# limix/CellRegMap

Hardware: AMD Instinct MI355X
Metric: variant-tests/sec (interaction test) (higher is better)
Workload: dtype f64

## Files before the change

cellregmap_amd/csrc/api_core.hip:

```cpp
#include <dlfcn.h>

#include <algorithm>
#include <atomic>
#include <cstdarg>
#include <mutex>

#include <map>

#include "crm_internal.h"
#include "eigh.h"

namespace crm {

static thread_local std::string g_error;

void set_error(const char* fmt, ...) {
    char buf[1024];
    va_list ap;
    va_start(ap, fmt);
    vsnprintf(buf, sizeof buf, fmt, ap);
    va_end(ap);
    g_error = buf;
}

// ... 220 lines not shown
}

int crm_ctx_synchronize(crm_ctx* c) {
    return crm::guarded_on("crm_ctx_synchronize", c, [&]() -> int {
    if (!c) return CRM_ERR_ARG;
    CRM_HIP(hipSetDevice(c->device));
    CRM_HIP(hipStreamSynchronize(c->stream));
    return CRM_OK;
    });
}

int crm_set_block_variants(crm_ctx* c, int variants) {
    return crm::guarded_on("crm_set_block_variants", c, [&]() -> int {
    if (!c || variants < 0) return CRM_ERR_ARG;
    c->block_variants = variants == 0 ? 0 : (int)round_up(variants, 128);
    return CRM_OK;
    });
}

int crm_set_null_fit_polish(crm_ctx* c, int on) {
    return crm::guarded_on("crm_set_null_fit_polish", c, [&]() -> int {
    if (!c) return CRM_ERR_ARG;
    c->polish = on != 0;
    return CRM_OK;
    });
}

int crm_set_progress_callback(crm_ctx* c, void (*callback)(long, long, void*), void* user) {
    return crm::guarded_on("crm_set_progress_callback", c, [&]() -> int {
    if (!c) return CRM_ERR_ARG;
    if (callback) c->progress[std::this_thread::get_id()] = crm_ctx::Progress{callback, user};
    else c->progress.erase(std::this_thread::get_id());
    return CRM_OK;
    });
}

int crm_set_fast_rotation(crm_ctx* c, int on) {
    return crm::guarded_on("crm_set_fast_rotation", c, [&]() -> int {
    if (!c) return CRM_ERR_ARG;
    c->fast_T = on != 0;
    return CRM_OK;
    });
}

extern "C++" {
namespace crm {
namespace {
struct FormSlot { const char* name; int value; bool set; };
FormSlot g_forms[] = {{"gram_staged", 0, false}, {"kr_no_tail", 0, false}, {"nullfit_per_wave", 0, false}, {"kin_fold", 0, false},
                      {"eigh_one_stage", 0, false}, {"nullfit_exact", 0, false}, {"donor_pairs", 0, false},
                      {"pairs_without_kinship_term", 0, false}, {"flat_kappa_milli", 0, false}, {"chase_abort", 0, false}, {"nullfit_one_per_wave", 0, false},
                      {"kin_diag", 0, false}, {"donor_pairs_rotate", 0, false}, {"rho0_positions", 0, false},
                      {"rotation_tails", 0, false}, {"woodbury_ytY", 0, false},
                      {"wb_block_order", 0, false}, {"block_fused", 0, false}, {"wb_gram_fused", 0, false}};
std::mutex g_forms_mu;
}
int form(const char* name, int otherwise) {
    std::lock_guard<std::mutex> lock(g_forms_mu);
    for (const FormSlot& f : g_forms)
        if (strcmp(f.name, name) == 0) return f.set ? f.value : otherwise;
    return otherwise;
}
}
}

int crm_test_set_form(const char* name, int value, int reset) {
    return crm::guarded("crm_test_set_form", [&]() -> int {
    if (!name) return CRM_ERR_ARG;
    std::lock_guard<std::mutex> lock(crm::g_forms_mu);
    for (crm::FormSlot& f : crm::g_forms)
        if (strcmp(f.name, name) == 0) {
            f.value = value;
            f.set = reset == 0;
            return CRM_OK;
        }
    crm::set_error("crm_test_set_form: no kernel form is called '%s'", name);
    return CRM_ERR_ARG;
    });
}

long crm_test_tail_launches(const crm_ctx* ctx) { return ctx ? ctx->tail_launches : -1; }

long crm_test_spectrum_tail_launches(const crm_ctx* ctx) { return ctx ? ctx->spectrum_tail_launches : -1; }

long crm_test_dense_repeats(const crm_ctx* ctx) { return ctx ? ctx->dense_repeats : -1; }

long crm_test_donor_pair_blocks(const crm_ctx* ctx) { return ctx ? ctx->donor_pair_blocks : -1; }

int crm_test_gram_dma_launches(const crm_ctx* ctx, long* launches) {
    return crm::guarded("crm_test_gram_dma_launches", [&]() -> int {
    if (!ctx || !launches) return CRM_ERR_ARG;
    *launches = ctx->gram_dma_launches;
    return CRM_OK;
    });
}
int crm_test_unrelated_donor_blocks(const crm_ctx* ctx, long* blocks) {
    return crm::guarded("crm_test_unrelated_donor_blocks", [&]() -> int {
    if (!ctx || !blocks) return CRM_ERR_ARG;
    *blocks = ctx->unrelated_donor_blocks;
    return CRM_OK;
    });
}

int crm_test_fused_blocks(const crm_ctx* ctx, long* blocks) {
    return crm::guarded("crm_test_fused_blocks", [&]() -> int {
    if (!ctx || !blocks) return CRM_ERR_ARG;
    *blocks = ctx->fused_blocks;
// ... 346 lines not shown
```

cellregmap_amd/csrc/assemble.hip:

```cpp
#include <type_traits>

#include "nullfit.h"

namespace crm {

namespace {

constexpr int CH = 64;
constexpr int SLD = 66;

typedef double v4d __attribute__((ext_vector_type(4)));

template <int NTL, int NG = 1>
__global__ __launch_bounds__(256) void gram_ext_kernel(AssembleArgs a, double* __restrict__ Gext, int KT) {
    constexpr int ROWS = 16 * NTL, NTILES = NTL * (NTL + 1) / 2, NLOC = (NTILES + NG - 1) / NG, MAXT = (NLOC + 3) / 4,
                  RPT = ROWS / 4;
    extern __shared__ double Ss[];
    __shared__ int tile_ij[NTILES];
    __shared__ const double* tail_ptr[ROWS];
    const int b = blockIdx.x;
    const NullFitOut fit = a.fit[b];
    const AssembleRho R = a.rho[fit.rho_index];
    const int r = R.r;
    const double ratio = fit.v0 / fit.v1;
    const long pos = a.sorted_pos[b];
    const double* __restrict__ Arows = pos >= 0 ? a.A + pos * a.k0 * a.ldA : a.A_none;
    const long a_stride = pos >= 0 ? a.ldA : 0;
    const int tid = threadIdx.x;
    const int lane = tid & 63, wave = tid >> 6;
    const int l15 = lane & 15, lq = lane >> 4;
    const int k0 = a.k0, c = a.c;

    for (int e = tid; e < NTILES; e += 256) {
        int ti = 0, rem = e;
        while (rem >= NTL - ti) { rem -= NTL - ti; ti++; }
        tile_ij[e] = ti | ((ti + rem) << 8);
    }
    for (int t = tid; t < KT - k0; t += 256) {
        const double* p;
        if (t < c) p = R.tW + (long)t * R.ldW;
        else if (t == c) p = R.T + (long)b * R.ldT;
        else if (t == c + 1) p = R.ty;
        else p = a.wb_R + (long)(t - c - 2) * a.wb_ldR;
        tail_ptr[t] = p;
    }
    __syncthreads();
    const int grp = NG > 1 ? (int)blockIdx.y : 0;
    const int first = (wave + b) & 3;
    const int nloc = (NTILES - grp + NG - 1) / NG;
    const int ntw = (nloc - first + 3) / 4;
    int t_i[MAXT], t_j[MAXT];
#pragma unroll
    for (int t = 0; t < MAXT; t++) {
        const int idx = grp + NG * (first + 4 * t);
        const int ij = tile_ij[idx < NTILES ? idx : 0];
// ... 231 lines not shown
        const int buf = ch & 1;
        if (ch + 1 < nchunks) {
            issue(ch + 1, buf ^ 1);
            weights(ch + 1, buf ^ 1);
        }
        chunk_mma(buf);
        __syncthreads();
    }
    double* const red = Ss + (wave & 1) * NTILES * 256;
    if (wave >= 2) {
#pragma unroll
        for (int t = 0; t < NTILES; t++)
#pragma unroll
            for (int reg = 0; reg < 4; reg++) red[(t * 4 + reg) * 64 + lane] = acc[t][reg];
    }
    __syncthreads();
    if (wave < 2) {
#pragma unroll
        for (int t = 0; t < NTILES; t++)
#pragma unroll
            for (int reg = 0; reg < 4; reg++) acc[t][reg] += red[(t * 4 + reg) * 64 + lane];
    }
    __syncthreads();
    if (wave == 1) {
#pragma unroll
        for (int t = 0; t < NTILES; t++)
#pragma unroll
            for (int reg = 0; reg < 4; reg++) red[(t * 4 + reg) * 64 + lane] = acc[t][reg];
    }
    __syncthreads();
    if (wave != 0) return;
    double* __restrict__ out = Gext + (long)b * KT * KT;
    int idx = 0;
#pragma unroll
    for (int ti = 0; ti < NTL; ti++) {
#pragma unroll
        for (int tj = ti; tj < NTL; tj++, idx++) {
#pragma unroll
            for (int reg = 0; reg < 4; reg++) {
                const double v = acc[idx][reg] + (Ss + NTILES * 256)[(idx * 4 + reg) * 64 + lane];
                const int row = 16 * ti + lq + 4 * reg, col = 16 * tj + l15;
                if (row < KT && col < KT) {
                    out[(long)row * KT + col] = v;
                    if (ti != tj) out[(long)col * KT + row] = v;
                }
            }
        }
    }
}

constexpr int GRAM_WCH = 32;
constexpr int gram_dma_wide_lds_doubles(int ntl) { return 2 * (16 * ((ntl + 3) / 4)) * GRAM_QLD + 4 * GRAM_WCH; }

template <int NTL>
__global__ __launch_bounds__(256, NTL <= 8 ? 2 : 1) void gram_ext_dma_wide_kernel(AssembleArgs a, double* __restrict__ Gext,
                                                                                  int KT) {
    constexpr int WCH = GRAM_WCH;
    constexpr int SLOTS = 16 * ((NTL + 3) / 4);
    constexpr int NTILES = NTL * (NTL + 1) / 2, MAXT = (NTILES + 3) / 4;
    constexpr int QLD = GRAM_QLD;
    constexpr int BUF = SLOTS * QLD;
    static_assert(gram_dma_wide_lds_doubles(NTL) == 2 * BUF + 4 * WCH, "the launch allocates what the kernel lays out");
    constexpr int IPW = SLOTS / 4;
    extern __shared__ double Ss[];
    double* const dS = Ss + 2 * BUF;
    const int b = blockIdx.x;
    const NullFitOut fit = a.fit[b];
    const AssembleRho R = a.rho[fit.rho_index];
    const int r = R.r;
    const double ratio = fit.v0 / fit.v1;
    const long pos = a.sorted_pos[b];
    const double* __restrict__ Arows = pos >= 0 ? a.A + pos * a.k0 * a.ldA : a.A_none;
    const long a_stride = pos >= 0 ? a.ldA : 0;
    const int tid = threadIdx.x;
    const int lane = tid & 63, wave = __builtin_amdgcn_readfirstlane(tid >> 6);
    const int l15 = lane & 15, lq = lane >> 4;
    const int k0 = a.k0, c = a.c;

    auto row_ptr = [&](int row) -> const double* {
        if (row >= KT) row = 0;
        if (row < k0) return Arows + (long)row * a_stride;
        const int t = row - k0;
        if (t > c + 1) return a.wb_R + (long)(t - c - 2) * a.wb_ldR;
        return t < c ? R.tW + (long)t * R.ldW : (t == c ? R.T + (long)b * R.ldT : R.ty);
    };
    auto row_off = [](int row) { return (16 * (row >> 6) + (row & 15)) * QLD + ((row >> 4) & 3) * WCH; };
    gram_gptr_t src[IPW];
#pragma unroll
    for (int q = 0; q < IPW; q++) {
        const int slot = wave + 4 * q;
        src[q] = (gram_gptr_t)(row_ptr(64 * (slot >> 4) + 16 * lq + (slot & 15)) + 2 * l15);
    }
    const int first = (wave + b) & 3;
    const int ntw = (NTILES - first + 3) / 4;
    int t_i[MAXT], t_j[MAXT], t_ij[MAXT];
#pragma unroll
    for (int t = 0; t < MAXT; t++) {
        int ti = 0, rem = first + 4 * t < NTILES ? first + 4 * t : 0;
        while (rem >= NTL - ti) { rem -= NTL - ti; ti++; }
        t_ij[t] = ti | ((ti + rem) << 8);
        t_i[t] = row_off(16 * ti + l15) + lq;
        t_j[t] = row_off(16 * (ti + rem) + l15) + lq;
    }
    v4d acc[MAXT];
#pragma unroll
    for (int t = 0; t < MAXT; t++) acc[t] = (v4d){0.0, 0.0, 0.0, 0.0};

    const int nfull = r / WCH, nchunks = (r + WCH - 1) / WCH;
    double* const sS = dS + 2 * WCH;
    auto issue_s0 = [&](int ch) __attribute__((always_inline)) {
        if (wave == 0 && ch < nchunks) {
            const int j = ch * WCH + (lane >> 1);
            const float* s0 = reinterpret_cast<const float*>(R.S0 + (j < r ? j : r - 1)) + (lane & 1);
            __builtin_amdgcn_global_load_lds((const float __attribute__((address_space(1)))*)s0,
                                             (gram_lptr_t)(sS + (ch & 1) * WCH), 4, 0, 0);
        }
    };
    auto weights = [&](int ch, double s0) __attribute__((always_inline)) {
        const double s = ch * WCH + lane < r ? ratio * s0 : 0.0;
        dS[(ch & 1) * WCH + lane] = s / (1.0 + s);
    };
    auto issue = [&](int ch, int buf) __attribute__((always_inline)) {
        if (ch < nfull) {
#pragma unroll
            for (int q = 0; q < IPW; q++)
                gram_dma16(src[q] + (long)ch * WCH, Ss + buf * BUF + (wave + 4 * q) * QLD);
        } else {
            for (int e = tid; e < 16 * NTL * WCH; e += 256) {
                const int row = e / WCH, col = e - row * WCH;
                const int j = ch * WCH + col;
                Ss[buf * BUF + row_off(row) + col] = (j < r && row < KT) ? row_ptr(row)[j] : 0.0;
            }
        }
    };
    auto chunk_mma = [&](int buf, auto nt_tag) __attribute__((always_inline)) {
        constexpr int NT = decltype(nt_tag)::value;
        const double* __restrict__ S = Ss + buf * BUF;
        const double* __restrict__ D = dS + buf * WCH + lq;
        double fa[2][NT], fb[2][NT];
        {
            const double dk = D[0];
#pragma unroll
            for (int t = 0; t < NT; t++) {
                fa[0][t] = S[t_i[t]];
                fb[0][t] = S[t_j[t]] * dk;
            }
        }
#pragma unroll
        for (int ks = 0; ks < WCH / 4; ks++) {
            const int cur = ks & 1, nx = cur ^ 1;
            if (ks + 1 < WCH / 4) {
                const double dk = D[4 * (ks + 1)];
#pragma unroll
                for (int t = 0; t < NT; t++) {
                    fa[nx][t] = S[t_i[t] + 4 * (ks + 1)];
                    fb[nx][t] = S[t_j[t] + 4 * (ks + 1)] * dk;
                }
            }
#pragma unroll
            for (int t = 0; t < NT; t++)
                acc[t] = __builtin_amdgcn_mfma_f64_16x16x4f64(fa[cur][t], fb[cur][t], acc[t], 0, 0, 0);
        }
    };
    if (wave == 0 && lane < WCH) weights(0, lane < r ? R.S0[lane] : 0.0);
    issue_s0(1);
    issue(0, 0);
    __syncthreads();
    for (int ch = 0; ch < nchunks; ch++) {
        const int buf = ch & 1;
        if (ch + 1 < nchunks) {
            if (wave == 0 && lane < WCH) weights(ch + 1, sS[(buf ^ 1) * WCH + lane]);
            issue(ch + 1, buf ^ 1);
        }
        issue_s0(ch + 2);
        if (ntw == MAXT) chunk_mma(buf, std::integral_constant<int, MAXT>{});
        else chunk_mma(buf, std::integral_constant<int, MAXT - 1>{});
        __syncthreads();
    }
    double* __restrict__ out = Gext + (long)b * KT * KT;
#pragma unroll
    for (int t = 0; t < MAXT; t++) {
        if (t >= ntw) continue;
        const int ri = (t_ij[t] & 255) * 16, cj = (t_ij[t] >> 8) * 16;
#pragma unroll
        for (int reg = 0; reg < 4; reg++) {
            const int row = ri + lq + 4 * reg, col = cj + l15;
            if (row < KT && col < KT) {
                out[(long)row * KT + col] = acc[t][reg];
                if (ri != cj) out[(long)col * KT + row] = acc[t][reg];
            }
        }
    }
}

__global__ __launch_bounds__(256) void woodbury_kernel(AssembleArgs a, const double* __restrict__ Gw, int KT,
                                                       double* __restrict__ Gext) {
    extern __shared__ double wsm[];
    const int k1 = a.wb_k1, KW = KT + k1, k0 = a.k0, c = a.c;
    const int b = blockIdx.x, tid = threadIdx.x;
    const NullFitOut fit = a.fit[b];
    const double g = fit.v0 * a.rho[fit.rho_index].rho;
    const double inv = 1.0 / fit.v1;
    const double* __restrict__ G = Gw + (long)b * KW * KW;
    double* __restrict__ out = Gext + (long)b * KT * KT;
    if (!(g > 0.0)) {
        for (int e = tid; e < KT * KT; e += 256) out[e] = G[(long)(e / KT) * KW + e % KT];
        return;
    }
    double* ME = wsm;
    double* Cm = ME + KT * k1;
    double* Z = Cm + k1 * k1;
    const long pos = a.sorted_pos[b];
    for (int e = tid; e < KT * k1; e += 256) {
        const int u = e / k1, f = e - u * k1;
        double plain;
        if (u < k0) plain = pos >= 0 ? a.wb_E1X[(long)f * a.wb_ldE1X + pos * k0 + u] : 0.0;
        else if (u < k0 + c) plain = a.wb_E1yW[(long)f * a.wb_ldE1yW + 1 + (u - k0)];
        else if (u == k0 + c) plain = a.wb_E1g[(long)f * a.wb_ldE1g + b];
        else plain = a.wb_E1yW[(long)f * a.wb_ldE1yW];
        ME[e] = (u < k0 && pos < 0) ? 0.0 : (plain - G[(long)u * KW + KT + f]) * inv;
    }
    for (int e = tid; e < k1 * k1; e += 256) {
        const int i = e / k1, j = e - i * k1;
        Cm[e] = (i == j ? 1.0 : 0.0) + g * (a.wb_EE[e] - G[(long)(KT + i) * KW + KT + j]) * inv;
    }
    __syncthreads();
    for (int j = 0; j < k1; j++) {
        if (tid == 0) Cm[j * k1 + j] = sqrt(Cm[j * k1 + j]);
        __syncthreads();
        const double l = Cm[j * k1 + j];
// ... 296 lines not shown
#undef sol

}

size_t woodbury_lds_bytes(int KT, int k1) { return sizeof(double) * ((size_t)2 * KT * k1 + (size_t)k1 * k1); }

size_t assemble_rows_scratch_doubles(int variants, int k0, int c) {
    const size_t P = (size_t)c + 1;
    const size_t lds = sizeof(double) * (P * P + 3 * P + k0 + 2 * (size_t)k0 * P);
    return lds > 150 * 1024 ? (size_t)variants * 2 * k0 * P : 0;
}

int launch_assemble(hipStream_t st, const AssembleArgs& a, int variants, double* Gext, double* fin_rows,
                    long* dma_launches) {
    if (variants <= 0) return CRM_OK;
    const int KT0 = a.k0 + a.c + 2;
    const int KT = KT0 + (a.wb_k1 > 0 ? a.wb_k1 : 0);
    double* const Gfin = Gext;
    if (a.wb_k1 > 0) {
        if (KT > CRM_MAX_GRAM_ROWS || woodbury_lds_bytes(KT0, a.wb_k1) > 150 * 1024 || !a.wb_Gw) {
            set_error("assemble: unrelated-donor form with %d + %d rows outside its supported range", KT0, a.wb_k1);
            return CRM_ERR_INTERNAL;
        }
        Gext = a.wb_Gw;
    }
    const int P = a.c + 1;
    const size_t fin_small = sizeof(double) * ((size_t)P * P + 3 * P + a.k0);
    size_t fin_lds = fin_small + sizeof(double) * 2 * (size_t)a.k0 * P;
    const bool rows_global = fin_lds > 150 * 1024;
    if (rows_global) fin_lds = fin_small;
    if (a.k0 > CRM_MAX_K0 || a.c > CRM_MAX_COV_XWIDE || KT > CRM_MAX_GRAM_ROWS || (rows_global && !fin_rows)) {
        set_error("assemble: k0=%d, c=%d outside the supported range (k0 <= %d, c <= %d, k0 + c + 2 <= %d)", a.k0, a.c,
                  CRM_MAX_K0, CRM_MAX_COV_XWIDE, CRM_MAX_GRAM_ROWS);
        return CRM_ERR_UNSUPPORTED;
    }
    const int ts = (KT + 15) / 16;
    const bool gram_done = a.wb_k1 > 0 && a.wb_gram_done != 0;
    bool dma = ts <= 9 && a.ldA % 2 == 0 && (reinterpret_cast<uintptr_t>(a.A) & 15) == 0 && !form("gram_staged", 0);
    for (int i = 0; dma && i < CRM_MAX_RHO; i++) {
        const AssembleRho& R = a.rho[i];
        if (R.r <= 0 && !R.ty) continue;
        dma = R.ldW % 2 == 0 && R.ldT % 2 == 0 && ((reinterpret_cast<uintptr_t>(R.ty) | reinterpret_cast<uintptr_t>(R.tW) |
                                                    reinterpret_cast<uintptr_t>(R.T)) & 15) == 0;
    }
    if (a.wb_k1 > 0) dma = dma && a.wb_ldR % 2 == 0 && (reinterpret_cast<uintptr_t>(a.wb_R) & 15) == 0;
#define CRM_GRAM_DMA(KERNEL, LDS_DOUBLES, NTL)                                                                \
    do {                                                                                                      \
        const size_t lds = sizeof(double) * LDS_DOUBLES(NTL);                                                 \
        if (lds > 60 * 1024)                                                                                  \
            CRM_HIP(hipFuncSetAttribute(reinterpret_cast<const void*>(&KERNEL<NTL>),                          \
                                        hipFuncAttributeMaxDynamicSharedMemorySize, (int)lds));               \
        hipLaunchKernelGGL(KERNEL<NTL>, dim3(variants), dim3(256), lds, st, a, Gext, KT);                     \
    } while (0)
#define CRM_GRAM_DMA_WIDE(NTL) CRM_GRAM_DMA(gram_ext_dma_wide_kernel, gram_dma_wide_lds_doubles, NTL)
    if (gram_done) {
    } else if (dma) {
        if (ts <= 2) CRM_GRAM_DMA(gram_ext_dma_kernel, gram_dma_lds_doubles, 2);
        else if (ts <= 4) CRM_GRAM_DMA(gram_ext_dma_kernel, gram_dma_lds_doubles, 4);
        else if (ts == 5) CRM_GRAM_DMA_WIDE(5);
        else if (ts == 6) CRM_GRAM_DMA_WIDE(6);
        else if (ts == 7) CRM_GRAM_DMA_WIDE(7);
        else if (ts == 8) CRM_GRAM_DMA_WIDE(8);
        else CRM_GRAM_DMA_WIDE(9);
    }
#undef CRM_GRAM_DMA_WIDE
#undef CRM_GRAM_DMA
#define CRM_GRAM(NTL)                                                                                         \
    do {                                                                                                      \
        const size_t lds = sizeof(double) * 16 * NTL * SLD;                                                   \
        if (lds > 60 * 1024)                                                                                  \
            CRM_HIP(hipFuncSetAttribute(reinterpret_cast<const void*>(&gram_ext_kernel<NTL>),                 \
                                        hipFuncAttributeMaxDynamicSharedMemorySize, (int)lds));               \
        hipLaunchKernelGGL(gram_ext_kernel<NTL>, dim3(variants), dim3(256), lds, st, a, Gext, KT);            \
    } while (0)
#define CRM_GRAM_GROUPS(NTL, NG)                                                                              \
    do {                                                                                                      \
        const size_t lds = sizeof(double) * 16 * NTL * SLD;                                                   \
        CRM_HIP(hipFuncSetAttribute(reinterpret_cast<const void*>(&gram_ext_kernel<NTL, NG>),                 \
                                    hipFuncAttributeMaxDynamicSharedMemorySize, (int)lds));                   \
        hipLaunchKernelGGL((gram_ext_kernel<NTL, NG>), dim3(variants, NG), dim3(256), lds, st, a, Gext, KT);  \
    } while (0)
    if (dma || gram_done) {
    } else if (ts <= 2) CRM_GRAM(2);
    else if (ts <= 4) CRM_GRAM(4);
    else if (ts <= 6) CRM_GRAM(6);
    else if (ts <= 7) CRM_GRAM(7);
    else if (ts <= 9) CRM_GRAM(9);
    else if (ts <= 12) CRM_GRAM_GROUPS(12, 2);
    else if (ts <= 15) CRM_GRAM_GROUPS(15, 4);
    else CRM_GRAM_GROUPS(18, 4);
#undef CRM_GRAM
#undef CRM_GRAM_GROUPS
    CRM_HIP(hipGetLastError());
    if ((dma || gram_done) && dma_launches) ++*dma_launches;
    const bool yty = a.wb_k1 > 0 && form("woodbury_ytY", 1) != 0;
    if (a.wb_k1 > 0) {
        const size_t lds = yty ? sizeof(double) * a.wb_k1 * (size_t)((KT0 + a.wb_k1) | 1) : woodbury_lds_bytes(KT0, a.wb_k1);
        const void* fn = yty ? reinterpret_cast<const void*>(&woodbury_yty_kernel) : reinterpret_cast<const void*>(&woodbury_kernel);
        if (lds > 60 * 1024) CRM_HIP(hipFuncSetAttribute(fn, hipFuncAttributeMaxDynamicSharedMemorySize, (int)lds));
        if (yty) hipLaunchKernelGGL(woodbury_yty_kernel, dim3(variants), dim3(256), lds, st, a, a.wb_Gw, KT0, Gfin);
        else hipLaunchKernelGGL(woodbury_kernel, dim3(variants), dim3(256), lds, st, a, a.wb_Gw, KT0, Gfin);
        CRM_HIP(hipGetLastError());
    }
    if (fin_lds > 60 * 1024)
        CRM_HIP(hipFuncSetAttribute(reinterpret_cast<const void*>(&finalize_kernel),
                                    hipFuncAttributeMaxDynamicSharedMemorySize, (int)fin_lds));
    hipLaunchKernelGGL(finalize_kernel, dim3(variants), dim3(128), fin_lds, st, a, Gfin, KT0, rows_global ? fin_rows : nullptr,
                       yty ? 1 : 0);
    CRM_HIP(hipGetLastError());
    return CRM_OK;
}

}
```

cellregmap_amd/csrc/tile_gram.h:

```cpp
#pragma once
#include <hip/hip_runtime.h>

namespace crm {

template <int TS, int CH, class Len, class Scale, class Value, class Sink>
__device__ inline double gram_tiles(double* S, double* sd, double* red, double* scal, int KT, Len len, bool by_row,
                                    Scale&& scale, Value&& value, Sink&& sink) {
    const int tid = threadIdx.x;
    const int ti = tid >> 4, tj = tid & 15;
    double acc[TS][TS];
#pragma unroll
    for (int i = 0; i < TS; i++)
#pragma unroll
        for (int j = 0; j < TS; j++) acc[i][j] = 0.0;
    double lpart = 0.0;
    constexpr int UNR = CH / 16;
    for (Len c0 = 0; c0 < len; c0 += CH) {
        if (tid < CH) sd[tid] = c0 + tid < len ? scale(c0, tid, lpart) : 0.0;
        __syncthreads();
        for (int e = tid; e < 16 * TS * CH; e += 256) {
            int row, q;
            if (by_row) { row = e / CH; q = e - row * CH; }
            else { q = e / (16 * TS); row = e - q * (16 * TS); }
            double v = 0.0;
            if (row < KT && c0 + q < len && sd[q] != 0.0) v = value(row, c0 + q) * sd[q];
            S[row * (CH + 1) + q] = v;
        }
        __syncthreads();
#pragma unroll UNR
        for (int q = 0; q < CH; q++) {
            double x[TS], y[TS];
#pragma unroll
            for (int i = 0; i < TS; i++) {
                x[i] = S[(ti + 16 * i) * (CH + 1) + q];
                y[i] = S[(tj + 16 * i) * (CH + 1) + q];
            }
#pragma unroll
            for (int i = 0; i < TS; i++)
#pragma unroll
                for (int j = 0; j < TS; j++) acc[i][j] += x[i] * y[j];
        }
        __syncthreads();
    }
#pragma unroll
    for (int i = 0; i < TS; i++) {
        const int row = ti + 16 * i;
#pragma unroll
        for (int j = 0; j < TS; j++) {
            const int col = tj + 16 * j;
            if (row < KT && col < KT) sink(row, col, acc[i][j]);
        }
    }
    if (!red) return 0.0;
    red[tid] = lpart;
    __syncthreads();
    if (tid == 0) {
        double s = 0.0;
        for (int i = 0; i < CH; i++) s += red[i];
        scal[1] = s;
    }
    __syncthreads();
    return scal[1];
}

__device__ inline int tri(int i, int k) { return i * (i + 1) / 2 + k; }
__device__ inline int tri_row(int e) {
    int i = (int)((sqrt(8.0 * e + 1.0) - 1.0) * 0.5);
    while (tri(i + 1, 0) <= e) i++;
    while (tri(i, 0) > e) i--;
    return i;
}

static __device__ bool packed_cholesky(double* H, int P, double* scal, double& logdet) {
    const int tid = threadIdx.x;
    logdet = 0.0;
    for (int j = 0; j < P; j++) {
        __syncthreads();
        if (tid == 0) {
            double d = H[tri(j, j)];
            for (int k = 0; k < j; k++) d -= H[tri(j, k)] * H[tri(j, k)];
            scal[0] = d;
        }
        __syncthreads();
        const double d = scal[0];
        if (!(d > 0.0)) return false;
        const double l = sqrt(d);
        logdet += 2.0 * log(l);
        for (int i = j + 1 + tid; i < P; i += blockDim.x) {
            double s = H[tri(i, j)];
            for (int k = 0; k < j; k++) s -= H[tri(i, k)] * H[tri(j, k)];
            H[tri(i, j)] = s / l;
        }
        if (tid == 0) H[tri(j, j)] = l;
        __syncthreads();
    }
    return true;
}

}
```

cellregmap_amd/csrc/wb_gram_fused.hip:

```cpp
#include <type_traits>

#include "nullfit.h"

namespace crm {

namespace {

typedef double v4d __attribute__((ext_vector_type(4)));
typedef const double __attribute__((address_space(1))) * fused_gptr_t;
typedef __attribute__((address_space(3))) void* fused_lptr_t;

__device__ __forceinline__ void fused_dma16(const double* src, double* lds_wave_uniform) {
    __builtin_amdgcn_global_load_lds((fused_gptr_t)src, (fused_lptr_t)lds_wave_uniform, 16, 0, 0);
}

__device__ __forceinline__ void dma_barrier() { asm volatile("s_waitcnt vmcnt(0) lgkmcnt(0)\n\ts_barrier" ::: "memory"); }

constexpr int WF_MAXQ_P = 10, WF_MAXQ_O = 9, WF_PSUM = 6;
constexpr int WF_UW = 56;

}

WbFusedLayout wb_gram_fused_layout(int k0, int KT, long ldp) {
    WbFusedLayout L;
    const int KS = (k0 + 3) / 4;
    L.urows = 4 * KS;
    L.UW = WF_UW;
    L.RS = (k0 + 4) | 2;
    L.nP = (int)(ldp / 128);
    L.nU = (L.urows * (L.UW / 2) + 63) / 64;
    L.rows_o = KT - k0;
    L.nO = (L.rows_o * (L.RS / 2) + 63) / 64;
    L.off_P = k0 * L.RS + L.nO * 128;
    L.off_U = L.off_P + L.nP * 128;
    L.off_S0 = L.off_U + L.nU * 128;
    L.off_d = L.off_S0 + 128;
    L.off_rp = L.off_d + 64;
    L.total = L.off_rp + ((L.rows_o + 1) & ~1);
    return L;
}

namespace {

template <int NTL>
__global__ __launch_bounds__(256, NTL <= 7 ? 2 : 1) void wb_gram_fused_kernel(AssembleArgs a, WbFusedArgs f, WbFusedLayout L, int KT) {
    constexpr int NTILES = NTL * (NTL + 1) / 2, MAXT = (NTILES + 3) / 4;
    extern __shared__ __align__(16) double smem[];
    double* const img = smem;
    double* const Pl = smem + L.off_P;
    double* const Ul = smem + L.off_U;
    double* const S0l = smem + L.off_S0;
    double* const dS = smem + L.off_d;
    const double** const rowp = reinterpret_cast<const double**>(smem + L.off_rp);
    const int b = blockIdx.x;
    const NullFitOut fit = a.fit[b];
    const AssembleRho R = a.rho[fit.rho_index];
    const double ratio = fit.v0 / fit.v1;
    const bool has_A = a.sorted_pos[b] >= 0;
    const int tid = threadIdx.x;
    const int lane = tid & 63, wave = __builtin_amdgcn_readfirstlane(tid >> 6);
    const int l15 = lane & 15, lq = lane >> 4;
    const int k0 = a.k0, c = a.c, RS = L.RS;
    constexpr int UW = WF_UW;
    const int npair = k0 * (k0 + 1) / 2, KS = (k0 + 3) / 4, JT = (k0 + 15) / 16;
    const int D = f.donors, Ptot = D * k0;
    const double* __restrict__ zeros = a.A_none;

    for (int e = tid; e < k0 * RS; e += 256) img[e] = 0.0;
    for (int t = tid; t < L.rows_o; t += 256) {
        const double* p;
        if (t < c) p = R.tW + (long)t * R.ldW;
        else if (t == c) p = R.T + (long)b * R.ldT;
        else if (t == c + 1) p = R.ty;
        else p = a.wb_R + (long)(t - c - 2) * a.wb_ldR;
        rowp[t] = p;
    }
    const int nPU = L.nP + L.nU + 1;
    int poff[WF_MAXQ_P], ocode[WF_MAXQ_O];
#pragma unroll
    for (int q = 0; q < WF_MAXQ_P; q++) {
        const int I = wave + 4 * q;
        if (I < L.nP) poff[q] = 128 * I + 2 * lane;
        else if (I < L.nP + L.nU) {
            const int u = 64 * (I - L.nP) + lane, k = u / (UW / 2), cu = u - k * (UW / 2);
            poff[q] = k < L.urows ? k * (int)f.ldu + 2 * cu : 0;
        } else poff[q] = 2 * lane;
    }
#pragma unroll
    for (int q = 0; q < WF_MAXQ_O; q++) {
        const int u = 64 * (wave + 4 * q) + lane, t = u / (RS / 2), cu = u - t * (RS / 2);
        ocode[q] = t < L.rows_o ? (t << 8) | (2 * cu) : -1;
    }
    auto chunk = [&](int d, int& start, int& end, int& c0, int& lim) __attribute__((always_inline)) {
        start = (k0 * d) & ~3;
        end = d + 1 < D ? (k0 * (d + 1)) & ~3 : (Ptot + 3) & ~3;
        c0 = 2 - (k0 * d - start);
        lim = end < Ptot ? end : Ptot;
    };
    auto issue_pus = [&](int d) __attribute__((always_inline)) {
        int start, end, c0, lim;
        chunk(d, start, end, c0, lim);
        const double* __restrict__ Pd = f.P + (size_t)d * f.p_slab + (long)b * f.ldp;
        const double* __restrict__ Ud = f.U + (size_t)d * f.u_slab;
        const double* __restrict__ S0 = R.S0 + (start - c0);
#pragma unroll
        for (int q = 0; q < WF_MAXQ_P; q++) {
            const int I = wave + 4 * q;
            if (I < L.nP) fused_dma16(Pd + poff[q], Pl + 128 * I);
            else if (I < L.nP + L.nU) fused_dma16(Ud + poff[q], Ul + 128 * (I - L.nP));
            else if (I < nPU) {
                const int col = poff[q];
                fused_dma16(col >= c0 && start - c0 + col < lim ? S0 + col : zeros, S0l);
            }
        }
    };
    auto issue_others = [&](int d) __attribute__((always_inline)) {
        int start, end, c0, lim;
        chunk(d, start, end, c0, lim);
        const int shift = start - c0;
#pragma unroll
        for (int q = 0; q < WF_MAXQ_O; q++) {
            const int I = wave + 4 * q;
            if (I < L.nO) {
                const int code = ocode[q], col = code & 255;
                const bool in = code >= 0 && col >= c0 && shift + col < lim;
                const double* src = zeros;
                if (in) src = rowp[code >> 8] + (shift + col);
                fused_dma16(src, img + k0 * RS + 128 * I);
            }
        }
    };
    const int iw = 16 * wave + l15;
    int pidx[16];
#pragma unroll
    for (int ks = 0; ks < 16; ks++) {
        const int k = 4 * ks + lq, lo = k < iw ? k : iw, hi = k < iw ? iw : k;
        pidx[ks] = k < k0 && iw < k0 ? lo * k0 - lo * (lo - 1) / 2 + (hi - lo) : 0;
    }
    const int first = (wave + b) & 3;
    const int ntw = (NTILES - first + 3) / 4;
    int t_i[MAXT], t_j[MAXT], t_ij[MAXT];
#pragma unroll
    for (int t = 0; t < MAXT; t++) {
        int ti = 0, rem = first + 4 * t < NTILES ? first + 4 * t : 0;
        while (rem >= NTL - ti) { rem -= NTL - ti; ti++; }
        t_ij[t] = ti | ((ti + rem) << 8);
        const int ri = 16 * ti + l15, rj = 16 * (ti + rem) + l15;
        t_i[t] = (ri < KT ? ri : 0) * RS + lq;
        t_j[t] = (rj < KT ? rj : 0) * RS + lq;
    }
    v4d acc[MAXT];
#pragma unroll
    for (int t = 0; t < MAXT; t++) acc[t] = (v4d){0.0, 0.0, 0.0, 0.0};
    double psum[WF_PSUM];
#pragma unroll
    for (int q = 0; q < WF_PSUM; q++) psum[q] = 0.0;
    const int per = (D + f.splits - 1) / f.splits;
    int split = 0;

    auto gram = [&](int col0, int nks, auto nt_tag) __attribute__((always_inline)) {
        constexpr int NT = decltype(nt_tag)::value;
        const double* __restrict__ S = img + col0;
        const double* __restrict__ Dw = dS + col0 + lq;
        double fa[NT], fr[NT];
        double dk = Dw[0];
#pragma unroll
        for (int t = 0; t < NT; t++) {
            fa[t] = S[t_i[t]];
            fr[t] = S[t_j[t]];
        }
        for (int ks = 0; ks < nks; ks++) {
            const bool more = ks + 1 < nks;
            const int nx = more ? 4 * (ks + 1) : 4 * ks;
            const double dn = Dw[nx];
#pragma unroll
            for (int t = 0; t < NT; t++) {
                acc[t] = __builtin_amdgcn_mfma_f64_16x16x4f64(fa[t], fr[t] * dk, acc[t], 0, 0, 0);
                fa[t] = S[t_i[t] + nx];
                fr[t] = S[t_j[t] + nx];
            }
            dk = dn;
        }
    };

    __syncthreads();
    issue_pus(0);
    issue_others(0);
    dma_barrier();
    for (int d = 0; d < D; d++) {
        int start, end, c0, lim;
        chunk(d, start, end, c0, lim);
        if (tid < RS) {
#pragma clang fp contract(off)
            const double s = ratio * S0l[tid];
            dS[tid] = s / (1.0 + s);
        }
#pragma unroll
        for (int q = 0; q < WF_PSUM; q++)
            if (tid + 256 * q < npair) psum[q] += Pl[tid + 256 * q];
        if (d + 1 == D || d + 1 == (split + 1) * per) {
            double* __restrict__ out = f.Psum + (size_t)split * f.psum_slab + (long)b * f.ldp;
#pragma unroll
            for (int q = 0; q < WF_PSUM; q++)
                if (tid + 256 * q < npair) { out[tid + 256 * q] = psum[q]; psum[q] = 0.0; }
            split++;
        }
        if (has_A && wave < JT) {
            unsigned uo = (unsigned)(lq * UW + l15);
            asm volatile("" : "+v"(uo));
            const double* __restrict__ ub = Ul + uo;
            const int jcut = end - k0 * d;
#pragma unroll
            for (int th = 0; th < 4; th += 2) {
                if (th < JT) {
                    v4d cr[2];
#pragma unroll
                    for (int t = 0; t < 2; t++) cr[t] = (v4d){0.0, 0.0, 0.0, 0.0};
                    double af[3], bf[3][2];
                    auto frag = [&](int ks, int slot) __attribute__((always_inline)) {
                        af[slot] = Pl[pidx[ks]];
#pragma unroll
                        for (int t = 0; t < 2; t++)
                            if (th + t < JT) bf[slot][t] = ub[4 * ks * UW + 16 * (th + t)];
                    };
                    frag(0, 0);
                    if (1 < KS) frag(1, 1);
#pragma unroll
                    for (int ks = 0; ks < 16; ks++) {
                        if (ks < KS) {
                            if (ks + 2 < KS) frag(ks + 2, (ks + 2) % 3);
#pragma unroll
                            for (int t = 0; t < 2; t++)
                                if (th + t < JT)
                                    cr[t] = __builtin_amdgcn_mfma_f64_16x16x4f64(af[ks % 3], bf[ks % 3][t], cr[t], 0, 0, 0);
                            __builtin_amdgcn_sched_barrier(0);
                        }
                    }
#pragma unroll
                    for (int reg = 0; reg < 4; reg++) {
                        const int r = 16 * wave + lq + 4 * reg;
                        if (r < k0) {
#pragma unroll
                            for (int t = 0; t < 2; t++) {
                                const int j = 16 * (th + t) + l15;
                                if (th + t < JT && j < k0) img[r * RS + (j < jcut ? j + 2 : j - jcut)] = cr[t][reg];
                            }
                        }
                    }
                }
            }
        }
        dma_barrier();
        if (d + 1 < D) issue_pus(d + 1);
        const int nks = (end - start) / 4;
        if (ntw == MAXT) gram(c0, nks, std::integral_constant<int, MAXT>{});
        else gram(c0, nks, std::integral_constant<int, MAXT - 1>{});
        dma_barrier();
        if (d + 1 < D) issue_others(d + 1);
    }
    for (; split < f.splits; split++) {
        double* __restrict__ out = f.Psum + (size_t)split * f.psum_slab + (long)b * f.ldp;
        for (int e = tid; e < npair; e += 256) out[e] = 0.0;
    }
    double* __restrict__ out = a.wb_Gw + (long)b * KT * KT;
#pragma unroll
    for (int t = 0; t < MAXT; t++) {
        if (t >= ntw) continue;
        const int ri = (t_ij[t] & 255) * 16, cj = (t_ij[t] >> 8) * 16;
#pragma unroll
        for (int reg = 0; reg < 4; reg++) {
            const int row = ri + lq + 4 * reg, col = cj + l15;
            if (row < KT && col < KT) {
                out[(long)row * KT + col] = acc[t][reg];
                if (ri != cj) out[(long)col * KT + row] = acc[t][reg];
            }
        }
    }
}

bool aligned16(const void* p) { return (reinterpret_cast<uintptr_t>(p) & 15) == 0; }

}

bool wb_gram_fused_serves(const AssembleArgs& a, const WbFusedArgs& f, int nrho) {
    const int k0 = a.k0, KT = k0 + a.c + 2 + a.wb_k1, ts = (KT + 15) / 16;
    if (form("wb_gram_fused", 1) == 0 || form("gram_staged", 0) != 0) return false;
    if (a.wb_k1 <= 0 || k0 % 2 != 0 || !donor_pairs_rotate_serves(k0) || ts < 5 || ts > 8 || f.donors < 1 || f.splits < 1) return false;
    if (f.ldp % 128 != 0 || f.ldp < k0 * (k0 + 1) / 2 || f.p_slab % 2 != 0 || f.u_slab % 2 != 0 || f.ldu % 2 != 0 || f.ldu < 4 * ((k0 + 3) / 4) ||
        f.k2pad < 4 * ((k0 + 3) / 4) || !aligned16(f.P) || !aligned16(f.U) || !aligned16(a.A_none) || !a.wb_Gw)
        return false;
    if (a.wb_ldR % 2 != 0 || !aligned16(a.wb_R)) return false;
    for (int i = 0; i < nrho; i++) {
        const AssembleRho& R = a.rho[i];
        if (R.r != f.donors * k0 || R.ldW % 2 != 0 || R.ldT % 2 != 0 || !aligned16(R.ty) || !aligned16(R.tW) || !aligned16(R.T) ||
            !aligned16(R.S0))
            return false;
    }
    const WbFusedLayout L = wb_gram_fused_layout(k0, KT, f.ldp);
    return L.nP + L.nU + 1 <= 4 * WF_MAXQ_P && L.nO <= 4 * WF_MAXQ_O && L.RS <= 64 && k0 * (k0 + 1) / 2 <= 256 * WF_PSUM &&
           sizeof(double) * (size_t)L.total <= 160 * 1024;
}

int launch_wb_gram_fused(hipStream_t st, const AssembleArgs& a, const WbFusedArgs& f, int nrho, int variants) {
    if (variants <= 0) return CRM_OK;
    if (!wb_gram_fused_serves(a, f, nrho)) {
        set_error("fused unrelated-donor Gram: k0=%d, c=%d outside the supported range", a.k0, a.c);
        return CRM_ERR_INTERNAL;
    }
    const int KT = a.k0 + a.c + 2 + a.wb_k1, ts = (KT + 15) / 16;
    const WbFusedLayout L = wb_gram_fused_layout(a.k0, KT, f.ldp);
    const size_t lds = sizeof(double) * (size_t)L.total;
#define CRM_WB_FUSED(NTL)                                                                                             \
    do {                                                                                                              \
        CRM_HIP(hipFuncSetAttribute(reinterpret_cast<const void*>(&wb_gram_fused_kernel<NTL>),                        \
                                    hipFuncAttributeMaxDynamicSharedMemorySize, (int)lds));                           \
        hipLaunchKernelGGL(wb_gram_fused_kernel<NTL>, dim3(variants), dim3(256), lds, st, a, f, L, KT);               \
    } while (0)
    if (ts == 5) CRM_WB_FUSED(5);
    else if (ts == 6) CRM_WB_FUSED(6);
    else if (ts == 7) CRM_WB_FUSED(7);
    else CRM_WB_FUSED(8);
#undef CRM_WB_FUSED
    CRM_HIP(hipGetLastError());
    return CRM_OK;
}

}
```

Before: 78480.

## Assign Gram tiles to waves as column strips to reuse fragment loads

Replaces the round-robin dealing of upper-triangle Gram tiles across the four waves with compile-time strip assignments. Each wave mostly owns the tiles of one or two tile-columns, so it loads the shared column fragment and the weighted B fragment once and reuses them across several MFMAs. The row fragments are also loaded only for the rows the wave needs. This cuts LDS reads per MFMA in both the DMA-wide Gram kernel and the fused Woodbury Gram kernel. The cost is an uneven per-wave tile count, more template instantiations, and register pressure from holding per-row fragments. A form flag keeps the old path available.

```diff
diff --git a/cellregmap_amd/csrc/api_core.hip b/cellregmap_amd/csrc/api_core.hip
--- a/cellregmap_amd/csrc/api_core.hip
+++ b/cellregmap_amd/csrc/api_core.hip
@@ -296,7 +296,8 @@
                       {"pairs_without_kinship_term", 0, false}, {"flat_kappa_milli", 0, false}, {"chase_abort", 0, false}, {"nullfit_one_per_wave", 0, false},
                       {"kin_diag", 0, false}, {"donor_pairs_rotate", 0, false}, {"rho0_positions", 0, false},
                       {"rotation_tails", 0, false}, {"woodbury_ytY", 0, false},
-                      {"wb_block_order", 0, false}, {"block_fused", 0, false}, {"wb_gram_fused", 0, false}};
+                      {"wb_block_order", 0, false}, {"block_fused", 0, false}, {"wb_gram_fused", 0, false},
+                      {"gram_strips", 0, false}};
 std::mutex g_forms_mu;
 }
 int form(const char* name, int otherwise) {
diff --git a/cellregmap_amd/csrc/assemble.hip b/cellregmap_amd/csrc/assemble.hip
--- a/cellregmap_amd/csrc/assemble.hip
+++ b/cellregmap_amd/csrc/assemble.hip
@@ -1,6 +1,7 @@
 #include <type_traits>
 
 #include "nullfit.h"
+#include "tile_gram.h"
 
 namespace crm {
 
@@ -338,7 +339,7 @@
 constexpr int GRAM_WCH = 32;
 constexpr int gram_dma_wide_lds_doubles(int ntl) { return 2 * (16 * ((ntl + 3) / 4)) * GRAM_QLD + 4 * GRAM_WCH; }
 
-template <int NTL>
+template <int NTL, bool STRIPS>
 __global__ __launch_bounds__(256, NTL <= 8 ? 2 : 1) void gram_ext_dma_wide_kernel(AssembleArgs a, double* __restrict__ Gext,
                                                                                   int KT) {
     constexpr int WCH = GRAM_WCH;
@@ -378,10 +379,11 @@
         src[q] = (gram_gptr_t)(row_ptr(64 * (slot >> 4) + 16 * lq + (slot & 15)) + 2 * l15);
     }
     const int first = (wave + b) & 3;
-    const int ntw = (NTILES - first + 3) / 4;
+    const int ntw = !STRIPS ? (NTILES - first + 3) / 4
+                            : first == 0 ? kStripDeal<NTL>.n[0] : first == 1 ? kStripDeal<NTL>.n[1] : first == 2 ? kStripDeal<NTL>.n[2] : kStripDeal<NTL>.n[3];
     int t_i[MAXT], t_j[MAXT], t_ij[MAXT];
 #pragma unroll
-    for (int t = 0; t < MAXT; t++) {
+    for (int t = 0; t < (STRIPS ? 0 : MAXT); t++) {
         int ti = 0, rem = first + 4 * t < NTILES ? first + 4 * t : 0;
         while (rem >= NTL - ti) { rem -= NTL - ti; ti++; }
         t_ij[t] = ti | ((ti + rem) << 8);
@@ -448,6 +450,32 @@
                 acc[t] = __builtin_amdgcn_mfma_f64_16x16x4f64(fa[cur][t], fb[cur][t], acc[t], 0, 0, 0);
         }
     };
+    auto chunk_mma_strips = [&](int buf, auto role_tag) __attribute__((always_inline)) {
+        constexpr int ROLE = decltype(role_tag)::value;
+        constexpr int NT = kStripDeal<NTL>.n[ROLE];
+        const double* __restrict__ S = Ss + buf * BUF + l15 * QLD + lq;
+        const double* __restrict__ D = dS + buf * WCH + lq;
+        double fr[2][NTL], fw[2][NTL];
+        auto fragments = [&](int set, int ks) __attribute__((always_inline)) {
+            const double dk = D[4 * ks];
+            static_for<0, NTL>([&](auto ic) {
+                constexpr int i = decltype(ic)::value;
+                if constexpr (kStripDeal<NTL>.reads(ROLE, i)) {
+                    fr[set][i] = S[16 * (i >> 2) * QLD + (i & 3) * WCH + 4 * ks];
+                    if constexpr (kStripDeal<NTL>.is_b(ROLE, i)) fw[set][i] = fr[set][i] * dk;
+                }
+            });
+        };
+        fragments(0, 0);
+        static_for<0, WCH / 4>([&](auto kc) {
+            constexpr int ks = decltype(kc)::value, cur = ks & 1;
+            if constexpr (ks + 1 < WCH / 4) fragments(cur ^ 1, ks + 1);
+            static_for<0, NT>([&](auto tc) {
+                constexpr int t = decltype(tc)::value;
+                acc[t] = __builtin_amdgcn_mfma_f64_16x16x4f64(fr[cur][kStripDeal<NTL>.ti[ROLE][t]], fw[cur][kStripDeal<NTL>.tj[ROLE][t]], acc[t], 0, 0, 0);
+            });
+        });
+    };
     if (wave == 0 && lane < WCH) weights(0, lane < r ? R.S0[lane] : 0.0);
     issue_s0(1);
     issue(0, 0);
@@ -459,9 +487,24 @@
             issue(ch + 1, buf ^ 1);
         }
         issue_s0(ch + 2);
-        if (ntw == MAXT) chunk_mma(buf, std::integral_constant<int, MAXT>{});
-        else chunk_mma(buf, std::integral_constant<int, MAXT - 1>{});
+        if constexpr (STRIPS) {
+            if (first == 0) chunk_mma_strips(buf, std::integral_constant<int, 0>{});
+            else if (first == 1) chunk_mma_strips(buf, std::integral_constant<int, 1>{});
+            else if (first == 2) chunk_mma_strips(buf, std::integral_constant<int, 2>{});
+            else chunk_mma_strips(buf, std::integral_constant<int, 3>{});
+        } else {
+            if (ntw == MAXT) chunk_mma(buf, std::integral_constant<int, MAXT>{});
+            else chunk_mma(buf, std::integral_constant<int, MAXT - 1>{});
+        }
         __syncthreads();
+    }
+    if constexpr (STRIPS) {
+        static_for<0, MAXT>([&](auto tc) {
+            constexpr int t = decltype(tc)::value;
+            constexpr int i0 = kStripDeal<NTL>.ti[0][t], i1 = kStripDeal<NTL>.ti[1][t], i2 = kStripDeal<NTL>.ti[2][t], i3 = kStripDeal<NTL>.ti[3][t];
+            constexpr int j0 = kStripDeal<NTL>.tj[0][t], j1 = kStripDeal<NTL>.tj[1][t], j2 = kStripDeal<NTL>.tj[2][t], j3 = kStripDeal<NTL>.tj[3][t];
+            t_ij[t] = (first == 0 ? i0 : first == 1 ? i1 : first == 2 ? i2 : i3) | ((first == 0 ? j0 : first == 1 ? j1 : first == 2 ? j2 : j3) << 8);
+        });
     }
     double* __restrict__ out = Gext + (long)b * KT * KT;
 #pragma unroll
@@ -864,7 +907,20 @@
                                         hipFuncAttributeMaxDynamicSharedMemorySize, (int)lds));               \
         hipLaunchKernelGGL(KERNEL<NTL>, dim3(variants), dim3(256), lds, st, a, Gext, KT);                     \
     } while (0)
-#define CRM_GRAM_DMA_WIDE(NTL) CRM_GRAM_DMA(gram_ext_dma_wide_kernel, gram_dma_wide_lds_doubles, NTL)
+    const bool strips = form("gram_strips", 1) != 0;
+#define CRM_GRAM_DMA_WIDE_AS(NTL, STRIPS)                                                                     \
+    do {                                                                                                      \
+        const size_t lds = sizeof(double) * gram_dma_wide_lds_doubles(NTL);                                   \
+        if (lds > 60 * 1024)                                                                                  \
+            CRM_HIP(hipFuncSetAttribute(reinterpret_cast<const void*>(&gram_ext_dma_wide_kernel<NTL, STRIPS>), \
+                                        hipFuncAttributeMaxDynamicSharedMemorySize, (int)lds));               \
+        hipLaunchKernelGGL((gram_ext_dma_wide_kernel<NTL, STRIPS>), dim3(variants), dim3(256), lds, st, a, Gext, KT); \
+    } while (0)
+#define CRM_GRAM_DMA_WIDE(NTL)                                                                                \
+    do {                                                                                                      \
+        if (strips) CRM_GRAM_DMA_WIDE_AS(NTL, true);                                                          \
+        else CRM_GRAM_DMA_WIDE_AS(NTL, false);                                                                \
+    } while (0)
     if (gram_done) {
     } else if (dma) {
         if (ts <= 2) CRM_GRAM_DMA(gram_ext_dma_kernel, gram_dma_lds_doubles, 2);
@@ -876,6 +932,7 @@
         else CRM_GRAM_DMA_WIDE(9);
     }
 #undef CRM_GRAM_DMA_WIDE
+#undef CRM_GRAM_DMA_WIDE_AS
 #undef CRM_GRAM_DMA
 #define CRM_GRAM(NTL)                                                                                         \
     do {                                                                                                      \
diff --git a/cellregmap_amd/csrc/tile_gram.h b/cellregmap_amd/csrc/tile_gram.h
--- a/cellregmap_amd/csrc/tile_gram.h
+++ b/cellregmap_amd/csrc/tile_gram.h
@@ -1,5 +1,7 @@
 #pragma once
 #include <hip/hip_runtime.h>
+
+#include <type_traits>
 
 namespace crm {
 
@@ -63,6 +65,74 @@
     return scal[1];
 }
 
+struct StripSeg { int j, i0, i1; };
+struct StripDeal {
+    static constexpr int MAXN = 12;
+    int ntl;
+    int n[4];
+    int ti[4][MAXN], tj[4][MAXN];
+    constexpr bool is_b(int w, int row) const {
+        for (int t = 0; t < n[w]; t++)
+            if (tj[w][t] == row) return true;
+        return false;
+    }
+    constexpr int last_a(int w, int row) const {
+        int last = -1;
+        for (int t = 0; t < n[w]; t++)
+            if (ti[w][t] == row) last = t;
+        return last;
+    }
+    constexpr bool reads(int w, int row) const { return is_b(w, row) || last_a(w, row) >= 0; }
+    constexpr bool valid() const {
+        const int maxt = (ntl * (ntl + 1) / 2 + 3) / 4;
+        for (int w = 0; w < 4; w++)
+            if (n[w] < 1 || n[w] > maxt) return false;
+        for (int i = 0; i < ntl; i++)
+            for (int j = i; j < ntl; j++) {
+                int seen = 0;
+                for (int w = 0; w < 4; w++)
+                    for (int t = 0; t < n[w]; t++) seen += ti[w][t] == i && tj[w][t] == j;
+                if (seen != 1) return false;
+            }
+        int total = 0;
+        for (int w = 0; w < 4; w++) total += n[w];
+        return total == ntl * (ntl + 1) / 2;
+    }
+};
+constexpr StripDeal make_strip_deal(int ntl, const StripSeg (&segs)[4][3]) {
+    StripDeal d{};
+    d.ntl = ntl;
+    for (int w = 0; w < 4; w++)
+        for (int s = 0; s < 3; s++)
+            for (int i = segs[w][s].i0; i < segs[w][s].i1; i++) {
+                d.ti[w][d.n[w]] = i;
+                d.tj[w][d.n[w]] = segs[w][s].j;
+                d.n[w]++;
+            }
+    return d;
+}
+template <int NTL> inline constexpr StripDeal kStripDeal = {};
+template <> inline constexpr StripDeal kStripDeal<5> =
+    make_strip_deal(5, {{{4, 0, 4}, {}, {}}, {{3, 0, 4}, {}, {}}, {{2, 0, 3}, {0, 0, 1}, {}}, {{1, 0, 2}, {4, 4, 5}, {}}});
+template <> inline constexpr StripDeal kStripDeal<6> =
+    make_strip_deal(6, {{{5, 0, 6}, {}, {}}, {{4, 0, 5}, {}, {}}, {{3, 0, 4}, {0, 0, 1}, {}}, {{2, 0, 3}, {1, 0, 2}, {}}});
+template <> inline constexpr StripDeal kStripDeal<7> =
+    make_strip_deal(7, {{{6, 0, 7}, {}, {}}, {{5, 0, 6}, {0, 0, 1}, {}}, {{4, 0, 5}, {1, 0, 2}, {}}, {{3, 0, 4}, {2, 0, 3}, {}}});
+template <> inline constexpr StripDeal kStripDeal<8> =
+    make_strip_deal(8, {{{7, 0, 8}, {0, 0, 1}, {}}, {{6, 0, 7}, {1, 0, 2}, {}}, {{5, 0, 6}, {2, 0, 3}, {}}, {{4, 0, 5}, {3, 0, 4}, {}}});
+template <> inline constexpr StripDeal kStripDeal<9> =
+    make_strip_deal(9, {{{8, 0, 9}, {1, 0, 2}, {0, 0, 1}}, {{7, 0, 8}, {2, 0, 3}, {}}, {{6, 0, 7}, {3, 0, 4}, {}}, {{5, 0, 6}, {4, 0, 5}, {}}});
+static_assert(kStripDeal<5>.valid() && kStripDeal<6>.valid() && kStripDeal<7>.valid() && kStripDeal<8>.valid() && kStripDeal<9>.valid(),
+              "a strip deal holds every tile of the upper triangle once and no role more than ceil(tiles / 4)");
+
+template <int I, int N, class F>
+__device__ __forceinline__ void static_for(F&& f) {
+    if constexpr (I < N) {
+        f(std::integral_constant<int, I>{});
+        static_for<I + 1, N>(f);
+    }
+}
+
 __device__ inline int tri(int i, int k) { return i * (i + 1) / 2 + k; }
 __device__ inline int tri_row(int e) {
     int i = (int)((sqrt(8.0 * e + 1.0) - 1.0) * 0.5);
diff --git a/cellregmap_amd/csrc/wb_gram_fused.hip b/cellregmap_amd/csrc/wb_gram_fused.hip
--- a/cellregmap_amd/csrc/wb_gram_fused.hip
+++ b/cellregmap_amd/csrc/wb_gram_fused.hip
@@ -1,6 +1,7 @@
 #include <type_traits>
 
 #include "nullfit.h"
+#include "tile_gram.h"
 
 namespace crm {
 
@@ -42,9 +43,10 @@
 
 namespace {
 
-template <int NTL>
+template <int NTL, bool STRIPS>
 __global__ __launch_bounds__(256, NTL <= 7 ? 2 : 1) void wb_gram_fused_kernel(AssembleArgs a, WbFusedArgs f, WbFusedLayout L, int KT) {
     constexpr int NTILES = NTL * (NTL + 1) / 2, MAXT = (NTILES + 3) / 4;
+    constexpr int MAXKS = 14;
     extern __shared__ __align__(16) double smem[];
     double* const img = smem;
     double* const Pl = smem + L.off_P;
@@ -138,10 +140,15 @@
         pidx[ks] = k < k0 && iw < k0 ? lo * k0 - lo * (lo - 1) / 2 + (hi - lo) : 0;
     }
     const int first = (wave + b) & 3;
-    const int ntw = (NTILES - first + 3) / 4;
-    int t_i[MAXT], t_j[MAXT], t_ij[MAXT];
-#pragma unroll
-    for (int t = 0; t < MAXT; t++) {
+    const int ntw = !STRIPS ? (NTILES - first + 3) / 4 : first == 0 ? kStripDeal<NTL>.n[0] : first == 1 ? kStripDeal<NTL>.n[1] : first == 2 ? kStripDeal<NTL>.n[2] : kStripDeal<NTL>.n[3];
+    int t_i[MAXT], t_j[MAXT], t_ij[MAXT], r_off[NTL];
+#pragma unroll
+    for (int i = 0; i < NTL; i++) {
+        const int row = 16 * i + l15;
+        r_off[i] = (row < KT ? row : 0) * RS + lq;
+    }
+#pragma unroll
+    for (int t = 0; t < (STRIPS ? 0 : MAXT); t++) {
         int ti = 0, rem = first + 4 * t < NTILES ? first + 4 * t : 0;
         while (rem >= NTL - ti) { rem -= NTL - ti; ti++; }
         t_ij[t] = ti | ((ti + rem) << 8);
@@ -181,6 +188,44 @@
             }
             dk = dn;
         }
+    };
+    auto gram_strips = [&](int col0, int nks, auto role_tag) __attribute__((always_inline)) {
+        constexpr int ROLE = decltype(role_tag)::value;
+        constexpr int NT = kStripDeal<NTL>.n[ROLE];
+        const double* __restrict__ S = img + col0;
+        const double* __restrict__ Dw = dS + col0 + lq;
+        const double* rows[NTL];
+        double fr[NTL], fw[NTL];
+        static_for<0, NTL>([&](auto ic) {
+            constexpr int i = decltype(ic)::value;
+            if constexpr (kStripDeal<NTL>.reads(ROLE, i)) {
+                rows[i] = S + r_off[i];
+                fr[i] = rows[i][0];
+            }
+        });
+        double dk = Dw[0];
+        auto step = [&](int off) __attribute__((always_inline)) {
+            static_for<0, NTL>([&](auto jc) {
+                constexpr int j = decltype(jc)::value;
+                if constexpr (kStripDeal<NTL>.is_b(ROLE, j)) {
+                    fw[j] = fr[j] * dk;
+                    if constexpr (kStripDeal<NTL>.last_a(ROLE, j) < 0) fr[j] = rows[j][off + 4];
+                }
+            });
+            static_for<0, NT>([&](auto tc) {
+                constexpr int t = decltype(tc)::value;
+                acc[t] = __builtin_amdgcn_mfma_f64_16x16x4f64(fr[kStripDeal<NTL>.ti[ROLE][t]], fw[kStripDeal<NTL>.tj[ROLE][t]], acc[t], 0, 0, 0);
+                static_for<0, NTL>([&](auto ic) {
+                    constexpr int i = decltype(ic)::value;
+                    if constexpr (kStripDeal<NTL>.last_a(ROLE, i) == t) fr[i] = rows[i][off + 4];
+                });
+            });
+            dk = Dw[off + 4];
+        };
+        static_for<0, MAXKS>([&](auto kc) {
+            constexpr int ks = decltype(kc)::value;
+            if (ks < nks) step(4 * ks);
+        });
     };
 
     __syncthreads();
@@ -253,8 +298,17 @@
         dma_barrier();
         if (d + 1 < D) issue_pus(d + 1);
         const int nks = (end - start) / 4;
-        if (ntw == MAXT) gram(c0, nks, std::integral_constant<int, MAXT>{});
-        else gram(c0, nks, std::integral_constant<int, MAXT - 1>{});
+        if constexpr (STRIPS) {
+            if (nks > 0) {
+                if (first == 0) gram_strips(c0, nks, std::integral_constant<int, 0>{});
+                else if (first == 1) gram_strips(c0, nks, std::integral_constant<int, 1>{});
+                else if (first == 2) gram_strips(c0, nks, std::integral_constant<int, 2>{});
+                else gram_strips(c0, nks, std::integral_constant<int, 3>{});
+            }
+        } else {
+            if (ntw == MAXT) gram(c0, nks, std::integral_constant<int, MAXT>{});
+            else gram(c0, nks, std::integral_constant<int, MAXT - 1>{});
+        }
         dma_barrier();
         if (d + 1 < D) issue_others(d + 1);
     }
@@ -263,6 +317,14 @@
         for (int e = tid; e < npair; e += 256) out[e] = 0.0;
     }
     double* __restrict__ out = a.wb_Gw + (long)b * KT * KT;
+    if constexpr (STRIPS) {
+        static_for<0, MAXT>([&](auto tc) {
+            constexpr int t = decltype(tc)::value;
+            constexpr int i0 = kStripDeal<NTL>.ti[0][t], i1 = kStripDeal<NTL>.ti[1][t], i2 = kStripDeal<NTL>.ti[2][t], i3 = kStripDeal<NTL>.ti[3][t];
+            constexpr int j0 = kStripDeal<NTL>.tj[0][t], j1 = kStripDeal<NTL>.tj[1][t], j2 = kStripDeal<NTL>.tj[2][t], j3 = kStripDeal<NTL>.tj[3][t];
+            t_ij[t] = (first == 0 ? i0 : first == 1 ? i1 : first == 2 ? i2 : i3) | ((first == 0 ? j0 : first == 1 ? j1 : first == 2 ? j2 : j3) << 8);
+        });
+    }
 #pragma unroll
     for (int t = 0; t < MAXT; t++) {
         if (t >= ntw) continue;
@@ -310,16 +372,23 @@
     const int KT = a.k0 + a.c + 2 + a.wb_k1, ts = (KT + 15) / 16;
     const WbFusedLayout L = wb_gram_fused_layout(a.k0, KT, f.ldp);
     const size_t lds = sizeof(double) * (size_t)L.total;
+    const bool strips = form("gram_strips", 1) != 0;
+#define CRM_WB_FUSED_AS(NTL, STRIPS)                                                                                  \
+    do {                                                                                                              \
+        CRM_HIP(hipFuncSetAttribute(reinterpret_cast<const void*>(&wb_gram_fused_kernel<NTL, STRIPS>),                \
+                                    hipFuncAttributeMaxDynamicSharedMemorySize, (int)lds));                           \
+        hipLaunchKernelGGL((wb_gram_fused_kernel<NTL, STRIPS>), dim3(variants), dim3(256), lds, st, a, f, L, KT);     \
+    } while (0)
 #define CRM_WB_FUSED(NTL)                                                                                             \
     do {                                                                                                              \
-        CRM_HIP(hipFuncSetAttribute(reinterpret_cast<const void*>(&wb_gram_fused_kernel<NTL>),                        \
-                                    hipFuncAttributeMaxDynamicSharedMemorySize, (int)lds));                           \
-        hipLaunchKernelGGL(wb_gram_fused_kernel<NTL>, dim3(variants), dim3(256), lds, st, a, f, L, KT);               \
+        if (strips) CRM_WB_FUSED_AS(NTL, true);                                                                       \
+        else CRM_WB_FUSED_AS(NTL, false);                                                                             \
     } while (0)
     if (ts == 5) CRM_WB_FUSED(5);
     else if (ts == 6) CRM_WB_FUSED(6);
     else if (ts == 7) CRM_WB_FUSED(7);
     else CRM_WB_FUSED(8);
+#undef CRM_WB_FUSED_AS
 #undef CRM_WB_FUSED
     CRM_HIP(hipGetLastError());
     return CRM_OK;
```

After: 80500, median of 6. 1.03x the previous value.
